# lppllppl920/EndoscopyDepthEstimation-Pytorch

Hardware: AMD Instinct MI355X
Metric: train frame-pairs/sec at 256x320 bs=8 (higher is better)
Workload: dtype f32

## Files before the change

endoscopydepthestimation-pytorch_amd/csrc/dgrad_newmap_kernels.h:

```cpp
#pragma once

#include "dgrad_block_kernels.h"

namespace endo {

template <int NL>
struct NewMapGeom {
    using G = DgradBlockGeom<1, 2, 3, 1, 4>;
    static constexpr int kStage = 12 * G::kCS;
    static constexpr int kW = 9 * 12 * 16;
    static constexpr int kWPre = (kW + kConvThreads - 1) / kConvThreads;
    static constexpr int kConsts = NL * 16 * 4;
    static constexpr size_t kBytes = sizeof(float) * (2 * kStage + NL * kW + kConsts);
    static constexpr int kBlocksPerCu = NL == 1 ? 4 : 3;
    static_assert(kBytes * kBlocksPerCu <= 160 * 1024, "LDS of the resident blocks");
    static_assert(sizeof(double) * 4 * NL * 16 * 2 <= sizeof(float) * kStage, "the final reduction aliases stage 0");
};

template <int NL>
__global__ void __launch_bounds__(kConvThreads, NewMapGeom<NL>::kBlocksPerCu) dgrad_newmap_kernel(const DgradBlockParams p, int tiles_y, int blocks_per_group, int tiles_per_block) {
    using NG = NewMapGeom<NL>;
    using G = typename NG::G;
    constexpr int R = 3;
    extern __shared__ __attribute__((aligned(16))) float smem[];
    float* s_g = smem;
    float* s_w = smem + 2 * NG::kStage;
    float* s_c = s_w + NL * NG::kW;

    const int tid = threadIdx.x;
    const int lane = tid & 63;
    const int wave = __builtin_amdgcn_readfirstlane(tid >> 6);
    const int li = lane & 15;
    const int lk = lane >> 4;
    const int wx = (wave & 1) * 16;
    const int wy = (wave >> 1) * R;

    const int gn = p.group_n > 0 ? p.group_n : p.n;
    const int tps = p.tiles_x * tiles_y;
    const int Q = static_cast<int>(gridDim.x >> 3);
    const bool interleave = (gridDim.x & 7) == 0 && Q > 0 && blocks_per_group % Q == 0;
    int grp, first, t_step, t_last;
    if (interleave) {
        const int lb0 = static_cast<int>(blockIdx.x & 7) * Q;
        grp = lb0 / blocks_per_group;
        const int b0 = lb0 - grp * blocks_per_group;
        first = b0 * tiles_per_block + static_cast<int>(blockIdx.x >> 3);
        t_last = min((b0 + Q) * tiles_per_block, tps * gn);
        t_step = Q;
    } else {
        const int lb = blockIdx.x;
        grp = lb / blocks_per_group;
        first = (lb - grp * blocks_per_group) * tiles_per_block;
        t_last = min(first + tiles_per_block, tps * gn);
        t_step = 1;
    }
    const int ntiles = first < t_last ? (t_last - first + t_step - 1) / t_step : 0;
    if (ntiles <= 0) return;
    const int64_t grp_off = p.group_n > 0 ? grp * p.gs : 0;

    struct Tile { int n, tx, ty, idx; };
    auto place = [&](Tile& t) {
        t.n = t.idx / tps;
        const int rem = t.idx - t.n * tps;
        t.ty = rem / p.tiles_x;
        t.tx = rem - t.ty * p.tiles_x;
    };
    auto advance = [&](Tile& t) { t.idx += t_step; place(t); };
    Tile cur;
    cur.idx = first;
    place(cur);

#pragma unroll
    for (int l = 0; l < NL; ++l) {
        const float* wl = p.wgt[l] + static_cast<int64_t>(p.w_ci_off) * 9;
        const int wcin = p.w_cin[l];
#pragma unroll
        for (int k = 0; k < NG::kWPre; ++k) {
            const int e0 = k * kConvThreads + wave * 64;
            if (e0 < NG::kW) {
                const int e = e0 + lane;
                const int j = e & 15, rest = e >> 4;
                const int tap = rest / 12, cc = rest - tap * 12;
                const bool ok = e < NG::kW && j < p.count;
                const float* src = ok ? wl + cc * 9 * wcin + j * 9 + (8 - tap) : g_pad_consts + 4;
                if (e < NG::kW) __builtin_amdgcn_global_load_lds((gptr_t)src, (lptr_t)(s_w + l * NG::kW + e0), 4, 0, 0);
            }
        }
    }
    const bool co_ok = li < p.count;
    if (tid < NL * 16) {
        const int l = tid >> 4, j = tid & 15;
        const float* sv = p.saved[0];
        const float* ga = p.gamma[0];
        const float* be = p.beta[0];
        if (NL > 1 && l == 1) { sv = p.saved[1]; ga = p.gamma[1]; be = p.beta[1]; }
        if (NL > 2 && l == 2) { sv = p.saved[2]; ga = p.gamma[2]; be = p.beta[2]; }
        f32x4 c4{0.f, 0.f, 0.f, 0.f};
        if (j < p.count) {
            const float mean = sv[grp_off + 2 * j], rstd = sv[grp_off + 2 * j + 1];
            c4 = f32x4{ga[j] * rstd, be[j], mean, rstd};
        }
        *reinterpret_cast<f32x4*>(s_c + tid * 4) = c4;
    }
    const float wfe = p.vg ? (co_ok ? p.vw[li] : 0.f) : 1.f;

    int u_ry[2], u_rx[2];
#pragma unroll
    for (int k = 0; k < 2; ++k) {
        const int u = lane + 64 * k;
        u_ry[k] = u / (G::kCols / 4);
        u_rx[k] = (u - u_ry[k] * (G::kCols / 4)) * 4;
    }
    const bool second_unit = lane + 64 < G::kUnits;
    const unsigned kOob = 0x80000000u;
    unsigned d_vo[2] = {kOob, kOob};
    const float* d_gn = p.g;
    auto dma_tile = [&](const Tile& t) {
        const int x0 = t.tx * G::kTileX, y0 = t.ty * G::kTileY;
#pragma unroll
        for (int k = 0; k < 2; ++k) {
            const int gy = y0 - 1 + u_ry[k], gx = x0 - G::kLeft + u_rx[k];
            const bool ok = gy >= 0 && gy < p.h && gx >= 0 && gx < p.w;
            d_vo[k] = ok ? 4u * static_cast<unsigned>(gy * p.g_w + gx) : kOob;
        }
        d_gn = p.g + grp_off + static_cast<int64_t>(t.n) * p.g_ns;
    };
    auto issue_chunk = [&](int l, int stage) {
        float* dst = s_g + stage * NG::kStage;
        const __amdgpu_buffer_rsrc_t gr = __builtin_amdgcn_make_buffer_rsrc(const_cast<float*>(d_gn), 0, NL * 12 * p.g_cs * 4, 0x00020000);
#pragma unroll
        for (int i = 0; i < 3; ++i) {
            const int c = wave + 4 * i;
            const unsigned so = 4u * static_cast<unsigned>((l * 12 + c) * p.g_cs);
            __builtin_amdgcn_raw_ptr_buffer_load_lds(gr, (lptr_t)(dst + c * G::kCS), 16, d_vo[0], so, 0, 0);
            if (second_unit) __builtin_amdgcn_raw_ptr_buffer_load_lds(gr, (lptr_t)(dst + c * G::kCS + 256), 16, d_vo[1], so, 0, 0);
        }
    };

    f32x4 xc[R], dc[R], total[R];
    const int lane_x = wx + 4 * lk;
    unsigned lo_r[R];
#pragma unroll
    for (int r = 0; r < R; ++r) lo_r[r] = static_cast<unsigned>(li * p.cs + (wy + r) * p.w + lane_x);
    const unsigned lo_ch = static_cast<unsigned>(li * p.cs);
    int64_t cur_off = 0, po_off = 0, cur_voff = 0;
    unsigned cur_rows = 0, po_rows = 0;
    bool cur_full = false, po_full = false;
    auto begin_tile = [&](const Tile& t) {
        const int x0 = t.tx * G::kTileX, y0 = t.ty * G::kTileY;
        cur_full = y0 + G::kTileY <= p.h && x0 + G::kTileX <= p.w;
        cur_off = grp_off + static_cast<int64_t>(t.n) * p.ns + y0 * p.w + x0;
        cur_voff = grp_off + static_cast<int64_t>(t.n) * p.cs + y0 * p.w + x0;
        const float* xb = p.x + cur_off;
        const float* ob = p.vg ? p.vg + cur_voff : p.out + cur_off;
        if (cur_full) {
            cur_rows = co_ok ? 7u : 0u;
#pragma unroll
            for (int r = 0; r < R; ++r) {
                xc[r] = *reinterpret_cast<const f32x4*>(xb + lo_r[r]);
                dc[r] = *reinterpret_cast<const f32x4*>(ob + (p.vg ? lo_r[r] - lo_ch : lo_r[r]));
            }
        } else {
            unsigned rows = 0;
#pragma unroll
            for (int r = 0; r < R; ++r)
                if (y0 + wy + r < p.h) rows |= 1u << r;
            cur_rows = (co_ok && x0 + lane_x + 3 < p.w) ? rows : 0u;
#pragma unroll
            for (int r = 0; r < R; ++r) {
                xc[r] = f32x4{0.f, 0.f, 0.f, 0.f};
                dc[r] = f32x4{0.f, 0.f, 0.f, 0.f};
                if (cur_rows & (1u << r)) {
                    xc[r] = *reinterpret_cast<const f32x4*>(xb + lo_r[r]);
                    dc[r] = *reinterpret_cast<const f32x4*>(ob + (p.vg ? lo_r[r] - lo_ch : lo_r[r]));
                }
            }
        }
    };

    auto store_results = [&]() {
        float* ob = p.out + po_off;
        if (po_full) {
            if (co_ok) {
#pragma unroll
                for (int r = 0; r < R; ++r) *reinterpret_cast<f32x4*>(ob + lo_r[r]) = dc[r];
            }
        } else {
#pragma unroll
            for (int r = 0; r < R; ++r)
                if (po_rows & (1u << r)) *reinterpret_cast<f32x4*>(ob + lo_r[r]) = dc[r];
        }
    };

    constexpr int kFlushTiles = 8;
    float fs1[NL], fs2[NL];
    double ds1[NL], ds2[NL];
    int tiles_since_flush = 0;
#pragma unroll
    for (int l = 0; l < NL; ++l) { fs1[l] = fs2[l] = 0.f; ds1[l] = ds2[l] = 0.0; }
    dma_tile(cur);
    issue_chunk(0, 0);
    Tile nxt = cur;
    advance(nxt);
    int stage = 0;

    for (int t = 0; t < ntiles; ++t) {
#pragma unroll
        for (int l = 0; l < NL; ++l) {
            asm volatile("s_waitcnt vmcnt(0)" ::: "memory");
            __syncthreads();
            if (l == 0) {
                if (t > 0) {
                    store_results();
                }
                begin_tile(cur);
            }
            if (l + 1 < NL) {
                issue_chunk(l + 1, stage ^ 1);
            } else if (t + 1 < ntiles) {
                dma_tile(nxt);
                issue_chunk(0, stage ^ 1);
            }
            f32x4 acc[R];
#pragma unroll
            for (int r = 0; r < R; ++r) acc[r] = f32x4{0.f, 0.f, 0.f, 0.f};
            {
                const float* sg = s_g + stage * NG::kStage;
                const float* wb = s_w + l * NG::kW;
                float av[2][3][R + 2], bw[2][9];
                auto load_quad = [&](int quad, int set) {
                    const float* a_base = sg + (quad * 4 + lk) * G::kCS + wy * G::kCols + wx + li + G::kColOff;
                    const float* b_base = wb + (quad * 4 + lk) * 16 + li;
#pragma unroll
                    for (int r = 0; r < R + 2; ++r)
#pragma unroll
                        for (int dx = 0; dx < 3; ++dx) av[set][dx][r] = a_base[r * G::kCols + dx];
#pragma unroll
                    for (int tap = 0; tap < 9; ++tap) bw[set][tap] = b_base[tap * 12 * 16];
                };
                load_quad(0, 0);
#pragma unroll
                for (int quad = 0; quad < 3; ++quad) {
                    const int set = quad & 1;
                    if (quad + 1 < 3) load_quad(quad + 1, set ^ 1);
                    __builtin_amdgcn_sched_barrier(0);
#pragma unroll
                    for (int dx = 0; dx < 3; ++dx)
#pragma unroll
                        for (int dy = 0; dy < 3; ++dy)
#pragma unroll
                            for (int r = 0; r < R; ++r)
                                acc[r] = __builtin_amdgcn_mfma_f32_16x16x4f32(av[set][dx][r + dy], bw[set][dy * 3 + dx], acc[r], 0, 0, 0);
                    __builtin_amdgcn_sched_barrier(0);
                }
            }
            {
                const f32x4 c4 = *reinterpret_cast<const f32x4*>(s_c + (l * 16 + li) * 4);
                const float scale = c4[0], beta = c4[1], mean = c4[2], rstd = c4[3];
                float s1 = 0.f, s2 = 0.f;
                auto row = [&](int r) {
#pragma unroll
                    for (int e = 0; e < 4; ++e) {
                        const float xcen = xc[r][e] - mean;
                        const float z = fmaf(xcen, scale, beta);
                        const float dz = z > 0.f ? acc[r][e] : 0.f;
                        s1 += dz;
                        s2 = fmaf(dz, xcen, s2);
                        total[r][e] = l == 0 ? scale * dz : fmaf(scale, dz, total[r][e]);
                    }
                };
                if (cur_full) {
#pragma unroll
                    for (int r = 0; r < R; ++r) row(r);
                } else {
#pragma unroll
                    for (int r = 0; r < R; ++r) {
                        if (l == 0) total[r] = f32x4{0.f, 0.f, 0.f, 0.f};
                        if (cur_rows & (1u << r)) row(r);
                    }
                }
                fs1[l] += s1;
                fs2[l] = fmaf(s2, rstd, fs2[l]);
            }
            if (l == NL - 1) {
#pragma unroll
                for (int r = 0; r < R; ++r)
#pragma unroll
                    for (int e = 0; e < 4; ++e) {
                        float old = dc[r][e] * wfe;
                        asm volatile("" : "+v"(old));
                        dc[r][e] = old + total[r][e];
                    }
                po_off = cur_off;
                po_rows = cur_rows;
                po_full = cur_full;
                cur = nxt;
                advance(nxt);
                if (++tiles_since_flush == kFlushTiles) {
                    tiles_since_flush = 0;
#pragma unroll
                    for (int k = 0; k < NL; ++k) {
                        ds1[k] += static_cast<double>(fs1[k]); ds2[k] += static_cast<double>(fs2[k]);
                        fs1[k] = 0.f; fs2[k] = 0.f;
                    }
                }
            }
            stage ^= 1;
            asm volatile("" : "+s"(stage));
        }
    }
    store_results();

    __syncthreads();
    double* red = reinterpret_cast<double*>(smem);
#pragma unroll
    for (int l = 0; l < NL; ++l) {
        double a = ds1[l] + static_cast<double>(fs1[l]), b = ds2[l] + static_cast<double>(fs2[l]);
        a += __shfl_xor(a, 16, 64); a += __shfl_xor(a, 32, 64);
        b += __shfl_xor(b, 16, 64); b += __shfl_xor(b, 32, 64);
        if (lk == 0) {
            red[((wave * NL + l) * 16 + li) * 2] = a;
            red[((wave * NL + l) * 16 + li) * 2 + 1] = b;
        }
    }
    __syncthreads();
    if (tid < 32 * NL) {
        const int l = tid >> 5, j = (tid >> 1) & 15, which = tid & 1;
        if (j < p.count) {
            double t = 0.0;
#pragma unroll
            for (int wv = 0; wv < 4; ++wv) t += red[((wv * NL + l) * 16 + j) * 2 + which];
            double* sc = p.scratch[0];
            if (NL > 1 && l == 1) sc = p.scratch[1];
            if (NL > 2 && l == 2) sc = p.scratch[2];
            atomicAdd(sc + bn_slot_offset(p.slot_stride) + grp_off / 2 + 2 * j + which, t);
        }
    }
}

inline bool dgrad_newmap_ok(const DgradBlockParams& p) {
    return p.count <= 16 && p.acc_from == 0 && 36ll * p.g_cs * 4 < (1ll << 31) && (16ll * p.cs + static_cast<int64_t>(p.h) * p.w) * 4 < (1ll << 32);
}

template <int NL>
inline int launch_dgrad_newmap(DgradBlockParams p, int cus, hipStream_t stream) {
    using NG = NewMapGeom<NL>;
    using G = typename NG::G;
    p.tiles_x = (p.w + G::kTileX - 1) / G::kTileX;
    const int tiles_y = (p.h + G::kTileY - 1) / G::kTileY;
    const int groups = p.group_n > 0 ? p.n / p.group_n : 1;
    const int tiles_per_group = p.tiles_x * tiles_y * (p.group_n > 0 ? p.group_n : p.n);
    const int resident = std::max(1, cus * NG::kBlocksPerCu / groups);
    const int tiles_per_block = (tiles_per_group + resident - 1) / resident;
    int blocks_per_group = (tiles_per_group + tiles_per_block - 1) / tiles_per_block;
    blocks_per_group = (blocks_per_group + 7) / 8 * 8;
    return launch_dyn(dgrad_newmap_kernel<NL>, dim3(groups * blocks_per_group), kConvThreads, NG::kBytes, stream, p, tiles_y, blocks_per_group, tiles_per_block);
}

}
```

endoscopydepthestimation-pytorch_amd/csrc/net.hip:

```cpp
#include <new>
#include <vector>

#include "dgrad_kernels.h"
#include "dgrad_block_kernels.h"
#include "dgrad_newmap_kernels.h"
#include "td_dgrad_kernels.h"
#include "td_fwd_kernels.h"
#include "wgrad_taps_kernels.h"
#include "wgrad1x1_kernels.h"
#include "wgrad_nsplit_kernels.h"
#include "wgrad_f34_kernels.h"
#include "wgrad_subpix_kernels.h"
#include "wino_fwd_kernels.h"
#include "wino4_fwd_kernels.h"
#include "dgrad_wino_kernels.h"
#include "dgrad_wino3_kernels.h"
#include "net_arch.h"

namespace endo {

int run_dgrad_wino3_nl4(const DgradBlockParams& p, const float* const* u, hipStream_t stream);
bool dgrad_wino3p_applies(const DgradBlockParams& p);
int run_dgrad_wino3p_nl4(const DgradBlockParams& p, const float* const* u, int blocks, double* fw_parts, int* blocks_used, hipStream_t stream);

constexpr int kSideStreamFromLevel = 0;

struct ConvP : ConvDesc { int64_t u = -1, ud = -1; };
using BnP = BnDesc;

struct Table : ModuleTable<ConvP> {
    WinoWeightTable wino;
    WinoWeightTable wino4;
    int64_t wino4_floats = 0;
    int64_t wino_floats = 0;
    WinoDgradTable wino_dgrad;
    int64_t wino_dgrad_floats = 0;
};

inline int level_channels(int level) { return level < kLevels ? 144 + down_in(level) : kBottIn + kNew; }

static const Table& table() {
    static Table* t = [] {
        Table* tb = new Table();
        WinoWeightTable& wt = tb->wino;
        WinoDgradTable& wd = tb->wino_dgrad;
        wt.layers = 0; wt.start[0] = 0;
        wd.layers = 0; wd.start[0] = 0;
        for (const ConvDesc& m : arch().convs) {
            if (!is_dense(m.role)) continue;
            ConvP& c = tb->conv(m);
            const int l = wt.layers++;
            c.u = tb->wino_floats;
            wt.cin[l] = c.cin; wt.cout[l] = c.cout; wt.w_off[l] = c.w; wt.u_off[l] = c.u;
            wt.start[l + 1] = wt.start[l] + c.cin * 16;
            tb->wino_floats += static_cast<int64_t>(c.cin) * kWinoUStride;
            wd.layers++;
            c.ud = tb->wino_dgrad_floats;
            wd.cin[l] = c.cin; wd.groups[l] = dense_base(m) / 16; wd.w_off[l] = c.w; wd.u_off[l] = c.ud;
            wd.start[l + 1] = wd.start[l] + 16 * wd.groups[l] * 12;
            tb->wino_dgrad_floats += static_cast<int64_t>(wd.groups[l]) * kWinoDgradSlice;
        }
        tb->wino4 = wt;
        for (int l = 0; l < wt.layers; ++l) { tb->wino4.u_off[l] = tb->wino4_floats; tb->wino4_floats += static_cast<int64_t>(wt.cin[l]) * kW4UStride; }
        return tb;
    }();
    return *t;
}

}

using namespace endo;

namespace endo { struct FwdPlan; struct BwdPlan; }

struct endo_net {
    int n, h, w;
    int groups;
    int64_t gs;
    struct Level { int h, w, t; int64_t plane; int64_t act, grad; int64_t sums; int64_t pq; } lv[kLevels + 1];
    int64_t pre_off;
    int64_t saved_off;
    int64_t idx_off[kLevels];
    int64_t sums_off;
    int64_t sums_bytes;
    int64_t tape_floats;
    int64_t partial_off;
    int64_t wino_off;
    int64_t wino4_off;
    int64_t pq_off;
    int64_t pq_floats;
    int64_t scratch_off;
    int64_t scratch_bytes;
    int64_t slot_stride;
    int64_t wg_scratch_off;
    int64_t tuw_scratch_off;
    int64_t wd_off;
    int64_t gplane_off;
    int64_t bias_parts_off;
    int64_t fw_parts_off;
    int64_t bias_parts_floats;
    int64_t gradws_floats;
    SideStream side;
    int opt[ENDO_OPT_COUNT];
    FwdPlan* last_fwd;
    BwdPlan* last_bwd;
};

namespace endo {


constexpr int kBiasPartChannels = 2048;
constexpr int kBiasPartLaunches = 64;
constexpr int kFwPartBlocks = 512;
struct BiasReduceTable {
    int n;
    struct Entry { const float* parts; float* bias; int count; int nparts; } e[kBiasPartLaunches];
};
struct BiasParts {
    BiasReduceTable table;
    int64_t used;
};

struct BnFin4 {
    const double* scratch[4];
    const float* saved[4];
    const float* gamma[4];
    float* ggamma[4];
    float* gbeta[4];
};

__global__ void __launch_bounds__(256) prep_dy_kernel(float* __restrict__ dbuf, const float* __restrict__ x, int64_t ns, int plane,
                                                      const float* __restrict__ pq_p, const float* __restrict__ pq_q,
                                                      float* bias_grad, int group_n, int64_t gs, const BnFin4 fin, int nl,
                                                      double count, int training, int64_t slot_stride,
                                                      const float* __restrict__ vg, const float* __restrict__ vw, float* __restrict__ parts) {
    __shared__ double scratch[4];
    const int c = blockIdx.y;
    const int grp = blockIdx.z / group_n, n = blockIdx.z - grp * group_n;
    float pc = pq_p[grp * gs + c], qc = pq_q[grp * gs + c];
    if (nl > 0) {
        const int64_t go = grp * gs;
        double dp = 0.0, dq = 0.0;
#pragma unroll
        for (int j = 0; j < 4; ++j) {
            if (j >= nl) break;
            const double s1 = bn_slot_sum(fin.scratch[j] + go / 2 + 2 * c, slot_stride);
            const double s2 = bn_slot_sum(fin.scratch[j] + go / 2 + 2 * c + 1, slot_stride);
            if (blockIdx.x == 0 && n == 0 && threadIdx.x == 0) {
                atomicAdd(fin.ggamma[j] + c, static_cast<float>(s2));
                atomicAdd(fin.gbeta[j] + c, static_cast<float>(s1));
            }
            if (training) {
                const double mean = fin.saved[j][go + 2 * c], rstd = fin.saved[j][go + 2 * c + 1];
                const double scale = fin.gamma[j][c] * rstd;
                const double k = scale * rstd * s2 / count;
                dp += static_cast<double>(static_cast<float>(-k));
                dq += static_cast<double>(static_cast<float>(-scale * s1 / count + k * mean));
            }
        }
        pc += static_cast<float>(dp);
        qc += static_cast<float>(dq);
    }
    const int64_t base = grp * gs + n * ns + static_cast<int64_t>(c) * plane;
    const float* vg_n = vg ? vg + grp * gs + static_cast<int64_t>(n) * plane : nullptr;
    const float wf = vg ? vw[c] : 0.f;
    float part = 0.f;
    if ((plane & 3) == 0 && !vg_n) {
        const int stride = gridDim.x * blockDim.x * 4;
        int i = (blockIdx.x * blockDim.x + threadIdx.x) * 4;
        for (; i + stride < plane; i += 2 * stride) {
            f32x4 g0 = *reinterpret_cast<const f32x4*>(dbuf + base + i);
            f32x4 g1 = *reinterpret_cast<const f32x4*>(dbuf + base + i + stride);
            const f32x4 x0 = *reinterpret_cast<const f32x4*>(x + base + i);
            const f32x4 x1 = *reinterpret_cast<const f32x4*>(x + base + i + stride);
#pragma unroll
            for (int e = 0; e < 4; ++e) { g0[e] += fmaf(pc, x0[e], qc); part += g0[e]; }
#pragma unroll
            for (int e = 0; e < 4; ++e) { g1[e] += fmaf(pc, x1[e], qc); part += g1[e]; }
            *reinterpret_cast<f32x4*>(dbuf + base + i) = g0;
            *reinterpret_cast<f32x4*>(dbuf + base + i + stride) = g1;
        }
        for (; i < plane; i += stride) {
            f32x4 g = *reinterpret_cast<const f32x4*>(dbuf + base + i);
            const f32x4 xv = *reinterpret_cast<const f32x4*>(x + base + i);
#pragma unroll
            for (int e = 0; e < 4; ++e) { g[e] += fmaf(pc, xv[e], qc); part += g[e]; }
            *reinterpret_cast<f32x4*>(dbuf + base + i) = g;
        }
    } else if ((plane & 3) == 0) {
        for (int i = (blockIdx.x * blockDim.x + threadIdx.x) * 4; i < plane; i += gridDim.x * blockDim.x * 4) {
            f32x4 g;
            if (vg_n) {
                const f32x4 gv = *reinterpret_cast<const f32x4*>(vg_n + i);
                g = f32x4{gv[0] * wf, gv[1] * wf, gv[2] * wf, gv[3] * wf};
            } else {
                g = *reinterpret_cast<const f32x4*>(dbuf + base + i);
            }
            const f32x4 xv = *reinterpret_cast<const f32x4*>(x + base + i);
#pragma unroll
            for (int e = 0; e < 4; ++e) { g[e] += fmaf(pc, xv[e], qc); part += g[e]; }
            *reinterpret_cast<f32x4*>(dbuf + base + i) = g;
        }
    } else {
        for (int i = blockIdx.x * blockDim.x + threadIdx.x; i < plane; i += gridDim.x * blockDim.x) {
            const float g = (vg_n ? vg_n[i] * wf : dbuf[base + i]) + fmaf(pc, x[base + i], qc);
            dbuf[base + i] = g;
            part += g;
        }
    }
    const int lane = threadIdx.x & 63, wave = threadIdx.x >> 6;
    double v = wave_sum(static_cast<double>(part));
    if (lane == 0) scratch[wave] = v;
    __syncthreads();
    if (threadIdx.x == 0 && bias_grad) {
        const float t = static_cast<float>(scratch[0] + scratch[1] + scratch[2] + scratch[3]);
        if (parts) parts[(static_cast<int64_t>(c) * gridDim.z + blockIdx.z) * gridDim.x + blockIdx.x] = t;
        else atomicAdd(bias_grad + c, t);
    }
}

__global__ void __launch_bounds__(256) bias_reduce_kernel(const BiasReduceTable tb) {
    const BiasReduceTable::Entry& e = tb.e[blockIdx.x];
    const int lane = threadIdx.x & 63, wave = threadIdx.x >> 6;
    for (int c = blockIdx.y * 4 + wave; c < e.count; c += gridDim.y * 4) {
        const float* src = e.parts + static_cast<int64_t>(c) * e.nparts;
        double t = 0.0;
        for (int i = lane; i < e.nparts; i += 64) t += static_cast<double>(src[i]);
        t = wave_sum(t);
        if (lane == 0) e.bias[c] += static_cast<float>(t);
    }
}

__global__ void bn_bwd_finalize_kernel(const double* __restrict__ scratch, const float* __restrict__ saved,
                                       const float* __restrict__ gamma, float* __restrict__ ggamma, float* __restrict__ gbeta,
                                       float* __restrict__ pq_p, float* __restrict__ pq_q, int c_count, double count, int training,
                                       int64_t gs, int64_t slot_stride) {
    scratch += blockIdx.y * (gs / 2); saved += blockIdx.y * gs; pq_p += blockIdx.y * gs; pq_q += blockIdx.y * gs;
    for (int c = blockIdx.x * blockDim.x + threadIdx.x; c < c_count; c += gridDim.x * blockDim.x) {
        const double s1 = bn_slot_sum(scratch + 2 * c, slot_stride), s2 = bn_slot_sum(scratch + 2 * c + 1, slot_stride);
        atomicAdd(ggamma + c, static_cast<float>(s2));
        atomicAdd(gbeta + c, static_cast<float>(s1));
        if (training) {
            const double mean = saved[2 * c], rstd = saved[2 * c + 1];
            const double scale = gamma[c] * rstd;
            const double k = scale * rstd * s2 / count;
            pq_p[c] += static_cast<float>(-k);
            pq_q[c] += static_cast<float>(-scale * s1 / count + k * mean);
        }
    }
}

__global__ void bn_bwd_finalize4_kernel(const BnFin4 a, int nl, float* __restrict__ pq_p, float* __restrict__ pq_q, int c_count, double count,
                                        int training, int64_t gs, int64_t slot_stride) {
    const int64_t go = blockIdx.y * gs;
    pq_p += go; pq_q += go;
    for (int c = blockIdx.x * blockDim.x + threadIdx.x; c < c_count; c += gridDim.x * blockDim.x) {
        double dp = 0.0, dq = 0.0;
#pragma unroll
        for (int j = 0; j < 4; ++j) {
            if (j >= nl) break;
            const double s1 = bn_slot_sum(a.scratch[j] + go / 2 + 2 * c, slot_stride);
            const double s2 = bn_slot_sum(a.scratch[j] + go / 2 + 2 * c + 1, slot_stride);
            atomicAdd(a.ggamma[j] + c, static_cast<float>(s2));
            atomicAdd(a.gbeta[j] + c, static_cast<float>(s1));
            if (training) {
                const double mean = a.saved[j][go + 2 * c], rstd = a.saved[j][go + 2 * c + 1];
                const double scale = a.gamma[j][c] * rstd;
                const double k = scale * rstd * s2 / count;
                dp += static_cast<double>(static_cast<float>(-k));
                dq += static_cast<double>(static_cast<float>(-scale * s1 / count + k * mean));
            }
        }
        if (training) {
            pq_p[c] += static_cast<float>(dp);
            pq_q[c] += static_cast<float>(dq);
        }
    }
}

__host__ __device__ inline void tu_tap_range(int r, int& k0, int& k1) { k0 = r == 2 ? 2 : 0; k1 = r == 0 ? 0 : 2; }

__global__ void tu_phase_weights_kernel(const float* __restrict__ w, int cout, int cin, float* __restrict__ out) {
    const int total = cin * kTuW9;
    for (int i = blockIdx.x * blockDim.x + threadIdx.x; i < total; i += gridDim.x * blockDim.x) {
        const int co = i % 48;
        const int rc = (i / 48) % 9;
        const int ci = i / kTuW9;
        float v = 0.f;
        if (co < cout) {
            const float* src = w + (static_cast<int64_t>(co) * cin + ci) * 9;
            int ky0, ky1, kx0, kx1;
            tu_tap_range(rc / 3, ky0, ky1);
            tu_tap_range(rc % 3, kx0, kx1);
            for (int ky = ky0; ky <= ky1; ++ky)
                for (int kx = kx0; kx <= kx1; ++kx) v += src[ky * 3 + kx];
        }
        out[i] = v;
    }
}

__global__ void tu_subpix_dgrad_weights_kernel(const float* __restrict__ w, int cout, int cin, float* __restrict__ out) {
    const int total = cout * kTuW9;
    for (int i = blockIdx.x * blockDim.x + threadIdx.x; i < total; i += gridDim.x * blockDim.x) {
        const int ci = i % 48;
        const int rc = (i / 48) % 9;
        const int co = i / kTuW9;
        float v = 0.f;
        if (ci < cin) {
            const float* src = w + (static_cast<int64_t>(co) * cin + ci) * 9;
            int ky0, ky1, kx0, kx1;
            tu_tap_range(rc / 3, ky0, ky1);
            tu_tap_range(rc % 3, kx0, kx1);
            for (int ky = ky0; ky <= ky1; ++ky)
                for (int kx = kx0; kx <= kx1; ++kx) v += src[ky * 3 + kx];
        }
        out[i] = v;
    }
}

__global__ void __launch_bounds__(256) finalize_partial_kernel(const float* __restrict__ partial, int64_t split_stride, int ksplit,
                                                               int64_t pns, int plane, const float* __restrict__ bias,
                                                               float* __restrict__ out, int64_t out_ns, double* out_sums,
                                                               int group_n, int64_t gs) {
    __shared__ double scratch[2 * 4];
    const int c = blockIdx.y;
    const int grp = blockIdx.z / group_n, n = blockIdx.z - grp * group_n;
    partial += grp * gs; out += grp * gs;
    if (out_sums) out_sums += grp * (gs / 2);
    const float b = bias[c];
    float part[2] = {0.f, 0.f};
    for (int i = blockIdx.x * blockDim.x + threadIdx.x; i < plane; i += gridDim.x * blockDim.x) {
        float v = b;
        for (int s = 0; s < ksplit; ++s) v += partial[s * split_stride + n * pns + static_cast<int64_t>(c) * plane + i];
        out[n * out_ns + static_cast<int64_t>(c) * plane + i] = v;
        part[0] += v;
        part[1] += v * v;
    }
    if (out_sums) block_sum_atomic<2>(part, out_sums + 2 * c, scratch);
}

__global__ void __launch_bounds__(256) final_fwd_kernel(const float* __restrict__ u, int64_t ns, int plane, int cin,
                                                        const float* __restrict__ wgt, const float* __restrict__ bias,
                                                        float* __restrict__ pre, float* __restrict__ out, int group_n, int64_t gs, int c_first) {
    __shared__ float s_w[192];
    for (int c = threadIdx.x; c < cin; c += blockDim.x) s_w[c] = wgt[c];
    __syncthreads();
    const int grp = blockIdx.y / group_n, n = blockIdx.y - grp * group_n;
    u += grp * gs;
    if (pre) pre += grp * gs;
    out += static_cast<int64_t>(grp) * group_n * plane;
    const bool vec = (plane & 3) == 0;
    if (vec) {
        for (int i = (blockIdx.x * blockDim.x + threadIdx.x) * 4; i < plane; i += gridDim.x * blockDim.x * 4) {
            f32x4 acc = {0.f, 0.f, 0.f, 0.f};
            if (c_first > 0) acc = *reinterpret_cast<const f32x4*>(pre + static_cast<int64_t>(n) * plane + i);
            const float* src = u + n * ns + i;
            for (int c = c_first; c < cin; ++c) {
                const f32x4 v = *reinterpret_cast<const f32x4*>(src + static_cast<int64_t>(c) * plane);
                const float wc = s_w[c];
                acc[0] = fmaf(v[0], wc, acc[0]); acc[1] = fmaf(v[1], wc, acc[1]);
                acc[2] = fmaf(v[2], wc, acc[2]); acc[3] = fmaf(v[3], wc, acc[3]);
            }
            const float b = bias[0];
            f32x4 o;
            for (int e = 0; e < 4; ++e) { acc[e] += b; o[e] = fabsf(acc[e]); }
            if (pre) *reinterpret_cast<f32x4*>(pre + static_cast<int64_t>(n) * plane + i) = acc;
            *reinterpret_cast<f32x4*>(out + static_cast<int64_t>(n) * plane + i) = o;
        }
    } else {
        for (int i = blockIdx.x * blockDim.x + threadIdx.x; i < plane; i += gridDim.x * blockDim.x) {
            float acc = c_first > 0 ? pre[static_cast<int64_t>(n) * plane + i] : 0.f;
            for (int c = c_first; c < cin; ++c) acc = fmaf(u[n * ns + static_cast<int64_t>(c) * plane + i], s_w[c], acc);
            acc += bias[0];
            if (pre) pre[static_cast<int64_t>(n) * plane + i] = acc;
            out[static_cast<int64_t>(n) * plane + i] = fabsf(acc);
        }
    }
}

__device__ __forceinline__ float sign_of(float v) { return v > 0.f ? 1.f : (v < 0.f ? -1.f : 0.f); }

__global__ void __launch_bounds__(256) final_g_kernel(const float* __restrict__ gout, const float* __restrict__ pre, float* __restrict__ g,
                                                      int plane, int group_n, int64_t gs) {
    const int grp = blockIdx.y / group_n, n = blockIdx.y - grp * group_n;
    gout += static_cast<int64_t>(blockIdx.y) * plane; pre += grp * gs + static_cast<int64_t>(n) * plane; g += grp * gs + static_cast<int64_t>(n) * plane;
    for (int i = blockIdx.x * blockDim.x + threadIdx.x; i < plane; i += gridDim.x * blockDim.x) g[i] = gout[i] * sign_of(pre[i]);
}

__global__ void __launch_bounds__(256) final_bwd_data_kernel(const float* __restrict__ gout, const float* __restrict__ pre,
                                                             const float* __restrict__ wgt, float* __restrict__ dbuf,
                                                             int64_t ns, int plane, int cin, int group_n, int64_t gs, int c_first) {
    __shared__ float s_w[192];
    for (int c = threadIdx.x; c < cin; c += blockDim.x) s_w[c] = wgt[c];
    __syncthreads();
    const int grp = blockIdx.y / group_n, n = blockIdx.y - grp * group_n;
    gout += static_cast<int64_t>(grp) * group_n * plane; pre += grp * gs; dbuf += grp * gs;
    for (int i = blockIdx.x * blockDim.x + threadIdx.x; i < plane; i += gridDim.x * blockDim.x) {
        const float g = gout[static_cast<int64_t>(n) * plane + i] * sign_of(pre[static_cast<int64_t>(n) * plane + i]);
        for (int c = c_first; c < cin; ++c) dbuf[n * ns + static_cast<int64_t>(c) * plane + i] = g * s_w[c];
    }
}

__global__ void __launch_bounds__(256) final_bwd_weight_kernel(const float* __restrict__ gout, const float* __restrict__ pre,
                                                               const float* __restrict__ u, int64_t ns, int plane, int cin,
                                                               int group_n, int64_t gs, float* __restrict__ gw, float* __restrict__ gb, int c_first) {
    __shared__ double scratch[4];
    const int c = c_first + blockIdx.x;
    const int grp = blockIdx.z / group_n, n = blockIdx.z - grp * group_n;
    const float* gp = gout + static_cast<int64_t>(blockIdx.z) * plane;
    const float* pp = pre + grp * gs + static_cast<int64_t>(n) * plane;
    const float* up = u + grp * gs + n * ns + static_cast<int64_t>(c < cin ? c : 0) * plane;
    float part = 0.f, part2 = 0.f;
    if ((plane & 3) == 0) {
        const int stride = gridDim.y * blockDim.x * 4;
        for (int i = (blockIdx.y * blockDim.x + threadIdx.x) * 4; i < plane; i += stride) {
            const f32x4 gv = *reinterpret_cast<const f32x4*>(gp + i);
            const f32x4 pv = *reinterpret_cast<const f32x4*>(pp + i);
            f32x4 uv = {1.f, 1.f, 1.f, 1.f};
            if (c < cin) uv = *reinterpret_cast<const f32x4*>(up + i);
            part += gv[0] * sign_of(pv[0]) * uv[0] + gv[1] * sign_of(pv[1]) * uv[1];
            part2 += gv[2] * sign_of(pv[2]) * uv[2] + gv[3] * sign_of(pv[3]) * uv[3];
        }
    } else {
        for (int i = blockIdx.y * blockDim.x + threadIdx.x; i < plane; i += gridDim.y * blockDim.x)
            part += gp[i] * sign_of(pp[i]) * (c < cin ? up[i] : 1.f);
    }
    const int lane = threadIdx.x & 63, wave = threadIdx.x >> 6;
    double v = wave_sum(static_cast<double>(part + part2));
    if (lane == 0) scratch[wave] = v;
    __syncthreads();
    if (threadIdx.x == 0) {
        const float t = static_cast<float>(scratch[0] + scratch[1] + scratch[2] + scratch[3]);
        if (c < cin) atomicAdd(gw + c, t); else atomicAdd(gb, t);
    }
}

__global__ void __launch_bounds__(64) final_w_reduce_kernel(const double* __restrict__ parts, int nblocks, int count, float* __restrict__ gw) {
    const int c = blockIdx.x;
    double t = 0.0;
    for (int b = threadIdx.x; b < nblocks; b += 64) t += parts[static_cast<int64_t>(b) * count + c];
    t = wave_sum(t);
    if (threadIdx.x == 0) atomicAdd(gw + c, static_cast<float>(t));
}

constexpr int kBlocks = 2 * kLevels + 1, kDense = kBlocks * kLayers;

enum class DenseFwd { Wino4, Wino2_32x16, Wino2_32x8, SplitK, Direct32x8, Direct16x8, DirectAuto };
struct FwdPlan {
    struct Dense {
        DenseFwd form;
        int ksplit;
        bool chunk_weights;
    } dense[kDense];
    bool bf16;
    bool wino4_weights;
    bool fuse_final;
    bool td_persistent[kLevels];
    bool tu_subpix[kLevels];
};

enum class NewMap { Bf16, Persistent, Vec16, Dword };
enum class BasePass { Block8, Block8Bf16, Wino3, Wino3Persistent, Wino8 };
enum class DenseWgrad { F34, NSplit, Taps, Direct };
enum class TdDgrad { Persistent, Runs128, Dma, Staged };
enum class TuWgrad { Subpix, Taps, Direct };
enum class TuDgrad { Subpix32x8, Subpix16x8, Subpix16x4, Plain };
enum class FirstWgrad { F34Prep, F34, Taps, Direct };
struct BwdPlan {
    struct Block {
        bool fused;
        NewMap newmap[kLayers];
        BasePass base;
// ... 1134 lines not shown
```

Measured before the change: 527.8.

## Deepen newmap dgrad DMA ring with counted vmcnt waits and quad-packed weights

Generalizes the newmap dgrad kernel to a configurable S-stage LDS ring, issuing the next chunk's DMA right after the barrier. It replaces the blanket vmcnt(0) wait with counted partial waits so activation loads and stores can stay in flight across chunks. Weights are re-laid out in LDS so each thread reads eight taps with two 16-byte loads plus one scalar, and results go through a separate total array. A 4x-unrolled loop is added to the BN-backward elementwise pass. The hand-counted vmcnt bookkeeping is fragile and could race if the counts are wrong, and the default S=2 keeps the same occupancy.

```diff
diff --git a/endoscopydepthestimation-pytorch_amd/csrc/dgrad_newmap_kernels.h b/endoscopydepthestimation-pytorch_amd/csrc/dgrad_newmap_kernels.h
--- a/endoscopydepthestimation-pytorch_amd/csrc/dgrad_newmap_kernels.h
+++ b/endoscopydepthestimation-pytorch_amd/csrc/dgrad_newmap_kernels.h
@@ -4,27 +4,47 @@
 
 namespace endo {
 
-template <int NL>
+template <int NL, int S = 2>
 struct NewMapGeom {
     using G = DgradBlockGeom<1, 2, 3, 1, 4>;
+    static constexpr int kStages = S;
     static constexpr int kStage = 12 * G::kCS;
-    static constexpr int kW = 9 * 12 * 16;
+    static constexpr int kWQ = 12 * 2 * 16 * 4;
+    static constexpr int kW = kWQ + 12 * 16;
     static constexpr int kWPre = (kW + kConvThreads - 1) / kConvThreads;
     static constexpr int kConsts = NL * 16 * 4;
-    static constexpr size_t kBytes = sizeof(float) * (2 * kStage + NL * kW + kConsts);
-    static constexpr int kBlocksPerCu = NL == 1 ? 4 : 3;
-    static_assert(kBytes * kBlocksPerCu <= 160 * 1024, "LDS of the resident blocks");
+    static constexpr size_t kBytes = sizeof(float) * (S * kStage + NL * kW + kConsts);
+    static constexpr int kBlocksPerCu = static_cast<int>(160 * 1024 / kBytes) < 4 ? static_cast<int>(160 * 1024 / kBytes) : 4;
+    static constexpr int kDmaOps = 6;
+    static_assert(S == 2 || S == 3, "ring depth");
+    static_assert(S != 2 || kBlocksPerCu == (NL == 1 ? 4 : 3), "LDS of the resident blocks");
+    static_assert((S * kStage) % 4 == 0 && kW % 4 == 0, "16-byte reads of the weight slices");
     static_assert(sizeof(double) * 4 * NL * 16 * 2 <= sizeof(float) * kStage, "the final reduction aliases stage 0");
 };
 
-template <int NL>
-__global__ void __launch_bounds__(kConvThreads, NewMapGeom<NL>::kBlocksPerCu) dgrad_newmap_kernel(const DgradBlockParams p, int tiles_y, int blocks_per_group, int tiles_per_block) {
-    using NG = NewMapGeom<NL>;
+__device__ __forceinline__ void newmap_wait_vm(int n) {
+#define ENDO_NM_WAIT(N) __builtin_amdgcn_s_waitcnt(((N) & 15) | 0x0070 | (((N) >> 4) << 14))
+    if (n >= 24) ENDO_NM_WAIT(24);
+    else if (n >= 21) ENDO_NM_WAIT(21);
+    else if (n >= 18) ENDO_NM_WAIT(18);
+    else if (n >= 15) ENDO_NM_WAIT(15);
+    else if (n >= 12) ENDO_NM_WAIT(12);
+    else if (n >= 9) ENDO_NM_WAIT(9);
+    else if (n >= 6) ENDO_NM_WAIT(6);
+    else if (n >= 3) ENDO_NM_WAIT(3);
+    else ENDO_NM_WAIT(0);
+#undef ENDO_NM_WAIT
+}
+
+template <int NL, int S = 2>
+__global__ void __launch_bounds__(kConvThreads, (NewMapGeom<NL, S>::kBlocksPerCu)) dgrad_newmap_kernel(const DgradBlockParams p, int tiles_y, int blocks_per_group, int tiles_per_block) {
+    using NG = NewMapGeom<NL, S>;
     using G = typename NG::G;
     constexpr int R = 3;
+    constexpr int D = S - 1;
     extern __shared__ __attribute__((aligned(16))) float smem[];
     float* s_g = smem;
-    float* s_w = smem + 2 * NG::kStage;
+    float* s_w = smem + S * NG::kStage;
     float* s_c = s_w + NL * NG::kW;
 
     const int tid = threadIdx.x;
@@ -59,13 +79,13 @@
     const int64_t grp_off = p.group_n > 0 ? grp * p.gs : 0;
 
     struct Tile { int n, tx, ty, idx; };
-    auto place = [&](Tile& t) {
+    auto place = [&](Tile& t) __attribute__((always_inline)) {
         t.n = t.idx / tps;
         const int rem = t.idx - t.n * tps;
         t.ty = rem / p.tiles_x;
         t.tx = rem - t.ty * p.tiles_x;
     };
-    auto advance = [&](Tile& t) { t.idx += t_step; place(t); };
+    auto advance = [&](Tile& t) __attribute__((always_inline)) { t.idx += t_step; place(t); };
     Tile cur;
     cur.idx = first;
     place(cur);
@@ -79,8 +99,11 @@
             const int e0 = k * kConvThreads + wave * 64;
             if (e0 < NG::kW) {
                 const int e = e0 + lane;
-                const int j = e & 15, rest = e >> 4;
-                const int tap = rest / 12, cc = rest - tap * 12;
+                const bool quads = e < NG::kWQ;
+                const int r8 = e - NG::kWQ;
+                const int j = quads ? (e >> 2) & 15 : r8 & 15;
+                const int cc = quads ? e >> 7 : r8 >> 4;
+                const int tap = quads ? ((e >> 6) & 1) * 4 + (e & 3) : 8;
                 const bool ok = e < NG::kW && j < p.count;
                 const float* src = ok ? wl + cc * 9 * wcin + j * 9 + (8 - tap) : g_pad_consts + 4;
                 if (e < NG::kW) __builtin_amdgcn_global_load_lds((gptr_t)src, (lptr_t)(s_w + l * NG::kW + e0), 4, 0, 0);
@@ -115,7 +138,7 @@
     const unsigned kOob = 0x80000000u;
     unsigned d_vo[2] = {kOob, kOob};
     const float* d_gn = p.g;
-    auto dma_tile = [&](const Tile& t) {
+    auto dma_tile = [&](const Tile& t) __attribute__((always_inline)) {
         const int x0 = t.tx * G::kTileX, y0 = t.ty * G::kTileY;
 #pragma unroll
         for (int k = 0; k < 2; ++k) {
@@ -125,7 +148,7 @@
         }
         d_gn = p.g + grp_off + static_cast<int64_t>(t.n) * p.g_ns;
     };
-    auto issue_chunk = [&](int l, int stage) {
+    auto issue_chunk = [&](int l, int stage) __attribute__((always_inline)) {
         float* dst = s_g + stage * NG::kStage;
         const __amdgpu_buffer_rsrc_t gr = __builtin_amdgcn_make_buffer_rsrc(const_cast<float*>(d_gn), 0, NL * 12 * p.g_cs * 4, 0x00020000);
 #pragma unroll
@@ -146,7 +169,7 @@
     int64_t cur_off = 0, po_off = 0, cur_voff = 0;
     unsigned cur_rows = 0, po_rows = 0;
     bool cur_full = false, po_full = false;
-    auto begin_tile = [&](const Tile& t) {
+    auto begin_tile = [&](const Tile& t) __attribute__((always_inline)) {
         const int x0 = t.tx * G::kTileX, y0 = t.ty * G::kTileY;
         cur_full = y0 + G::kTileY <= p.h && x0 + G::kTileX <= p.w;
         cur_off = grp_off + static_cast<int64_t>(t.n) * p.ns + y0 * p.w + x0;
@@ -156,10 +179,10 @@
         if (cur_full) {
             cur_rows = co_ok ? 7u : 0u;
 #pragma unroll
-            for (int r = 0; r < R; ++r) {
-                xc[r] = *reinterpret_cast<const f32x4*>(xb + lo_r[r]);
-                dc[r] = *reinterpret_cast<const f32x4*>(ob + (p.vg ? lo_r[r] - lo_ch : lo_r[r]));
-            }
+            for (int r = 0; r < R; ++r) xc[r] = *reinterpret_cast<const f32x4*>(xb + lo_r[r]);
+            __builtin_amdgcn_sched_barrier(0);
+#pragma unroll
+            for (int r = 0; r < R; ++r) dc[r] = *reinterpret_cast<const f32x4*>(ob + (p.vg ? lo_r[r] - lo_ch : lo_r[r]));
         } else {
             unsigned rows = 0;
 #pragma unroll
@@ -175,20 +198,21 @@
                     dc[r] = *reinterpret_cast<const f32x4*>(ob + (p.vg ? lo_r[r] - lo_ch : lo_r[r]));
                 }
             }
-        }
-    };
-
-    auto store_results = [&]() {
+            __builtin_amdgcn_s_waitcnt(0x0f70);
+        }
+    };
+
+    auto store_results = [&]() __attribute__((always_inline)) {
         float* ob = p.out + po_off;
         if (po_full) {
             if (co_ok) {
 #pragma unroll
-                for (int r = 0; r < R; ++r) *reinterpret_cast<f32x4*>(ob + lo_r[r]) = dc[r];
+                for (int r = 0; r < R; ++r) *reinterpret_cast<f32x4*>(ob + lo_r[r]) = total[r];
             }
         } else {
 #pragma unroll
             for (int r = 0; r < R; ++r)
-                if (po_rows & (1u << r)) *reinterpret_cast<f32x4*>(ob + lo_r[r]) = dc[r];
+                if (po_rows & (1u << r)) *reinterpret_cast<f32x4*>(ob + lo_r[r]) = total[r];
         }
     };
 
@@ -198,29 +222,51 @@
     int tiles_since_flush = 0;
 #pragma unroll
     for (int l = 0; l < NL; ++l) { fs1[l] = fs2[l] = 0.f; ds1[l] = ds2[l] = 0.0; }
-    dma_tile(cur);
-    issue_chunk(0, 0);
-    Tile nxt = cur;
-    advance(nxt);
+    int vm_tail = 0, vm_mid = 0, vm_since_d = 0;
+    Tile dpos = cur;
+    auto issue_next = [&](int dl, int st) __attribute__((always_inline)) {
+        if (dl == 0) dma_tile(dpos);
+        issue_chunk(dl, st);
+        if (dl == NL - 1) advance(dpos);
+    };
+    issue_next(0, 0);
+    if (D > 1 && 1 / NL < ntiles) {
+        issue_next(1 % NL, 1);
+        vm_mid = NG::kDmaOps;
+    }
     int stage = 0;
 
     for (int t = 0; t < ntiles; ++t) {
 #pragma unroll
         for (int l = 0; l < NL; ++l) {
-            asm volatile("s_waitcnt vmcnt(0)" ::: "memory");
-            __syncthreads();
+            newmap_wait_vm(D > 1 ? vm_mid + vm_tail : vm_tail);
+            __builtin_amdgcn_sched_barrier(0);
+            __builtin_amdgcn_s_barrier();
+            __builtin_amdgcn_sched_barrier(0);
+            int dma_ops = 0, tail = 0;
+            {
+                const int dl = (l + D) % NL, dt = (l + D) / NL;
+                if (t + dt < ntiles) {
+                    issue_next(dl, stage == 0 ? S - 1 : stage - 1);
+                    dma_ops = NG::kDmaOps;
+                }
+            }
+            __builtin_amdgcn_sched_barrier(0);
             if (l == 0) {
                 if (t > 0) {
                     store_results();
-                }
+                    if (po_full) tail += R;
+                }
+                __builtin_amdgcn_sched_barrier(0);
                 begin_tile(cur);
-            }
-            if (l + 1 < NL) {
-                issue_chunk(l + 1, stage ^ 1);
-            } else if (t + 1 < ntiles) {
-                dma_tile(nxt);
-                issue_chunk(0, stage ^ 1);
-            }
+                if (cur_full) tail += 2 * R;
+                vm_since_d = 0;
+            } else {
+                vm_since_d += dma_ops;
+            }
+            vm_mid = vm_tail + dma_ops;
+            vm_tail = tail;
+            __builtin_amdgcn_sched_barrier(0);
             f32x4 acc[R];
 #pragma unroll
             for (int r = 0; r < R; ++r) acc[r] = f32x4{0.f, 0.f, 0.f, 0.f};
@@ -228,15 +274,18 @@
                 const float* sg = s_g + stage * NG::kStage;
                 const float* wb = s_w + l * NG::kW;
                 float av[2][3][R + 2], bw[2][9];
-                auto load_quad = [&](int quad, int set) {
+                auto load_quad = [&](int quad, int set) __attribute__((always_inline)) {
                     const float* a_base = sg + (quad * 4 + lk) * G::kCS + wy * G::kCols + wx + li + G::kColOff;
-                    const float* b_base = wb + (quad * 4 + lk) * 16 + li;
+                    const int cc = quad * 4 + lk;
 #pragma unroll
                     for (int r = 0; r < R + 2; ++r)
 #pragma unroll
                         for (int dx = 0; dx < 3; ++dx) av[set][dx][r] = a_base[r * G::kCols + dx];
-#pragma unroll
-                    for (int tap = 0; tap < 9; ++tap) bw[set][tap] = b_base[tap * 12 * 16];
+                    const f32x4 b0 = *reinterpret_cast<const f32x4*>(wb + ((cc * 2) * 16 + li) * 4);
+                    const f32x4 b1 = *reinterpret_cast<const f32x4*>(wb + ((cc * 2 + 1) * 16 + li) * 4);
+#pragma unroll
+                    for (int e = 0; e < 4; ++e) { bw[set][e] = b0[e]; bw[set][4 + e] = b1[e]; }
+                    bw[set][8] = wb[NG::kWQ + cc * 16 + li];
                 };
                 load_quad(0, 0);
 #pragma unroll
@@ -254,11 +303,16 @@
                     __builtin_amdgcn_sched_barrier(0);
                 }
             }
+            if (l == 0) {
+                __builtin_amdgcn_sched_barrier(0);
+                newmap_wait_vm(NL > 1 && cur_full ? R : 0);
+                __builtin_amdgcn_sched_barrier(0);
+            }
             {
                 const f32x4 c4 = *reinterpret_cast<const f32x4*>(s_c + (l * 16 + li) * 4);
                 const float scale = c4[0], beta = c4[1], mean = c4[2], rstd = c4[3];
                 float s1 = 0.f, s2 = 0.f;
-                auto row = [&](int r) {
+                auto row = [&](int r) __attribute__((always_inline)) {
 #pragma unroll
                     for (int e = 0; e < 4; ++e) {
                         const float xcen = xc[r][e] - mean;
@@ -283,19 +337,23 @@
                 fs2[l] = fmaf(s2, rstd, fs2[l]);
             }
             if (l == NL - 1) {
+                if (NL > 1) {
+                    __builtin_amdgcn_sched_barrier(0);
+                    newmap_wait_vm(vm_since_d);
+                    __builtin_amdgcn_sched_barrier(0);
+                }
 #pragma unroll
                 for (int r = 0; r < R; ++r)
 #pragma unroll
                     for (int e = 0; e < 4; ++e) {
                         float old = dc[r][e] * wfe;
                         asm volatile("" : "+v"(old));
-                        dc[r][e] = old + total[r][e];
+                        total[r][e] = old + total[r][e];
                     }
                 po_off = cur_off;
                 po_rows = cur_rows;
                 po_full = cur_full;
-                cur = nxt;
-                advance(nxt);
+                advance(cur);
                 if (++tiles_since_flush == kFlushTiles) {
                     tiles_since_flush = 0;
 #pragma unroll
@@ -305,7 +363,7 @@
                     }
                 }
             }
-            stage ^= 1;
+            stage = stage + 1 == S ? 0 : stage + 1;
             asm volatile("" : "+s"(stage));
         }
     }
@@ -342,9 +400,9 @@
     return p.count <= 16 && p.acc_from == 0 && 36ll * p.g_cs * 4 < (1ll << 31) && (16ll * p.cs + static_cast<int64_t>(p.h) * p.w) * 4 < (1ll << 32);
 }
 
-template <int NL>
+template <int NL, int S = 2>
 inline int launch_dgrad_newmap(DgradBlockParams p, int cus, hipStream_t stream) {
-    using NG = NewMapGeom<NL>;
+    using NG = NewMapGeom<NL, S>;
     using G = typename NG::G;
     p.tiles_x = (p.w + G::kTileX - 1) / G::kTileX;
     const int tiles_y = (p.h + G::kTileY - 1) / G::kTileY;
@@ -354,7 +412,7 @@
     const int tiles_per_block = (tiles_per_group + resident - 1) / resident;
     int blocks_per_group = (tiles_per_group + tiles_per_block - 1) / tiles_per_block;
     blocks_per_group = (blocks_per_group + 7) / 8 * 8;
-    return launch_dyn(dgrad_newmap_kernel<NL>, dim3(groups * blocks_per_group), kConvThreads, NG::kBytes, stream, p, tiles_y, blocks_per_group, tiles_per_block);
+    return launch_dyn(dgrad_newmap_kernel<NL, S>, dim3(groups * blocks_per_group), kConvThreads, NG::kBytes, stream, p, tiles_y, blocks_per_group, tiles_per_block);
 }
 
 }
diff --git a/endoscopydepthestimation-pytorch_amd/csrc/net.hip b/endoscopydepthestimation-pytorch_amd/csrc/net.hip
--- a/endoscopydepthestimation-pytorch_amd/csrc/net.hip
+++ b/endoscopydepthestimation-pytorch_amd/csrc/net.hip
@@ -168,6 +168,19 @@
     if ((plane & 3) == 0 && !vg_n) {
         const int stride = gridDim.x * blockDim.x * 4;
         int i = (blockIdx.x * blockDim.x + threadIdx.x) * 4;
+        for (; i + 3 * static_cast<int64_t>(stride) < plane; i += 4 * stride) {
+            f32x4 g[4], xv[4];
+#pragma unroll
+            for (int k = 0; k < 4; ++k) g[k] = *reinterpret_cast<const f32x4*>(dbuf + base + i + k * stride);
+#pragma unroll
+            for (int k = 0; k < 4; ++k) xv[k] = *reinterpret_cast<const f32x4*>(x + base + i + k * stride);
+#pragma unroll
+            for (int k = 0; k < 4; ++k) {
+#pragma unroll
+                for (int e = 0; e < 4; ++e) { g[k][e] += fmaf(pc, xv[k][e], qc); part += g[k][e]; }
+                *reinterpret_cast<f32x4*>(dbuf + base + i + k * stride) = g[k];
+            }
+        }
         for (; i + stride < plane; i += 2 * stride) {
             f32x4 g0 = *reinterpret_cast<const f32x4*>(dbuf + base + i);
             f32x4 g1 = *reinterpret_cast<const f32x4*>(dbuf + base + i + stride);
```

New measurement: 532.3, median of 6. Within noise of the previous version (+0.8%).
